# ComputationalRobotics/cuADMM

Measured on NVIDIA B200. Metric: ADMM iterations/s, higher is better.
Workload: dtype f64

## Files before the change

### cuadmm_b200/csrc/dense.cu

```cuda
#include "dense.h"
#include <stdio.h>
#include <stdlib.h>
#include <algorithm>

namespace cuadmm {

static constexpr int GB_M = 64, GB_N = 64, GB_K = 16, GB_PAD = 4;

__device__ __forceinline__ void dmma_m8n8k4(double& c0, double& c1, double a, double b) {
    asm volatile("mma.sync.aligned.m8n8k4.row.col.f64.f64.f64.f64 {%0,%1}, {%2}, {%3}, {%0,%1};"
                 : "+d"(c0), "+d"(c1) : "d"(a), "d"(b));
}

template <bool TA, bool TB>
__global__ void __launch_bounds__(128) dgemm_kernel(int64_t m, int64_t n, int64_t k, double alpha,
                                                    const double* __restrict__ A, int64_t lda,
                                                    const double* __restrict__ B, int64_t ldb,
                                                    double beta, double* C, int64_t ldc, int shape) {
    if (shape == 1 && (int64_t)blockIdx.y * GB_N > (int64_t)blockIdx.x * GB_M + (GB_M - 1)) return;
    __shared__ double As[2][GB_K][GB_M + GB_PAD];
    __shared__ double Bs[2][GB_K][GB_N + GB_PAD];
    const int tid = threadIdx.x, lane = tid & 31, warp = tid >> 5;
    const int wm = (warp & 1) * 32, wn = (warp >> 1) * 32;
    const int64_t m0 = (int64_t)blockIdx.x * GB_M, n0 = (int64_t)blockIdx.y * GB_N;
// ... 108 lines not shown
            for (int t = j; t < i; ++t) s -= S[i][t] * I[t][j];
            I[i][j] = (i >= j) ? s / S[i][i] : 0.0;
        }
    }
    __syncthreads();
    for (int e = tid; e < nb * nb; e += 256) {
        const int i = e % nb, j = e / nb;
        if (i >= j) A[i + j * lda] = S[i][j];
        if (inv) inv[i + (int64_t)j * NB] = I[i][j];
    }
    if (tid == 0 && bad && info) atomicAdd(info, 1);
}

void potrf_lower(cudaStream_t st, int64_t n, double* A, int64_t lda, double* inv_diag, int* d_info, const double* pivot_floor) {
    DevBuf<double> tmp(std::max<int64_t>(n * NB, 1));
    DevBuf<double> inv_local;
    if (!inv_diag) { inv_local.alloc(std::max<int64_t>(n * NB, 1)); inv_diag = inv_local.p; }
    const size_t potf2_bytes = sizeof(double) * 2 * NB * (NB + 1);
    CUADMM_CUDA(cudaFuncSetAttribute((const void*)potf2_inv_kernel, cudaFuncAttributeMaxDynamicSharedMemorySize, (int)potf2_bytes));
    for (int64_t j = 0; j < n; j += NB) {
        const int nb = (int)std::min<int64_t>(NB, n - j);
        double* Ajj = A + j + j * lda;
        double* invj = inv_diag + j * NB;
        potf2_inv_kernel<<<1, 256, potf2_bytes, st>>>(nb, Ajj, lda, invj, d_info, (int)(j / NB), pivot_floor ? pivot_floor + j : nullptr);
        const int64_t below = n - j - nb;
        if (below > 0) {
            double* Aij = A + (j + nb) + j * lda;
            dgemm(st, false, true, below, nb, nb, 1.0, Aij, lda, invj, NB, 0.0, tmp.p, below);
            CUADMM_CUDA(cudaMemcpy2DAsync(Aij, sizeof(double) * lda, tmp.p, sizeof(double) * below,
                                          sizeof(double) * below, nb, cudaMemcpyDeviceToDevice, st));
            double* A22 = A + (j + nb) + (j + nb) * lda;
            dgemm(st, false, true, below, below, nb, -1.0, Aij, lda, Aij, lda, 1.0, A22, lda, 1);
        }
    }
    CUADMM_CUDA(cudaGetLastError());
    CUADMM_CUDA(cudaStreamSynchronize(st));
}

__global__ void copy_inv_block_kernel(int nb, const double* __restrict__ inv, double* X, int64_t ldx) {
    for (int e = threadIdx.x; e < nb * nb; e += blockDim.x) {
        const int i = e % nb, j = e / nb;
        X[i + j * ldx] = inv[i + (int64_t)j * NB];
    }
}

void trtri_lower(cudaStream_t st, int64_t n, const double* L, int64_t ldl, const double* inv_diag, double* X, int64_t ldx) {
    CUADMM_CUDA(cudaMemset2DAsync(X, sizeof(double) * ldx, 0, sizeof(double) * n, n, st));
    DevBuf<double> T(std::max<int64_t>((int64_t)NB * n, 1));
    for (int64_t i = 0; i < n; i += NB) {
        const int nb = (int)std::min<int64_t>(NB, n - i);
        const double* invi = inv_diag + i * NB;
        copy_inv_block_kernel<<<1, 256, 0, st>>>(nb, invi, X + i + i * ldx, ldx);
        if (i > 0) {
            dgemm(st, false, false, nb, i, i, 1.0, L + i, ldl, X, ldx, 0.0, T.p, NB, 2);
            dgemm(st, false, false, nb, i, nb, -1.0, invi, NB, T.p, NB, 0.0, X + i, ldx);
        }
    }
    CUADMM_CUDA(cudaGetLastError());
    CUADMM_CUDA(cudaStreamSynchronize(st));
}

__global__ void scatter_coo_kernel(int64_t nnz, const int32_t* __restrict__ r, const int32_t* __restrict__ c,
                                   const double* __restrict__ v, double* D, int64_t ld, int symmetric) {
    const int64_t e = (int64_t)blockIdx.x * blockDim.x + threadIdx.x;
    if (e >= nnz) return;
    D[r[e] + (int64_t)c[e] * ld] = v[e];
    if (symmetric && r[e] != c[e]) D[c[e] + (int64_t)r[e] * ld] = v[e];
}

__global__ void transpose_kernel(int64_t n, const double* __restrict__ in, double* __restrict__ out) {
    __shared__ double tile[32][33];
    const int64_t bx = (int64_t)blockIdx.x * 32, by = (int64_t)blockIdx.y * 32;
    for (int j = threadIdx.y; j < 32; j += blockDim.y) {
        const int64_t x = bx + threadIdx.x, y = by + j;
        if (x < n && y < n) tile[j][threadIdx.x] = in[x + y * n];
    }
    __syncthreads();
    for (int j = threadIdx.y; j < 32; j += blockDim.y) {
        const int64_t x = by + threadIdx.x, y = bx + j;
        if (x < n && y < n) out[x + y * n] = tile[threadIdx.x][j];
    }
}

__global__ void tile_occupancy_kernel(int64_t r, int nt, const double* __restrict__ A, int* __restrict__ flags) {
    const int I = blockIdx.y, J = blockIdx.x;
    int any = 0;
    for (int e = threadIdx.x; e < 64 * 64; e += blockDim.x) {
        const int64_t i = (int64_t)I * 64 + e / 64, j = (int64_t)J * 64 + e % 64;
        if (i < r && j < r && A[i * r + j] != 0.0) any = 1;
    }
    if (__syncthreads_or(any) && threadIdx.x == 0) flags[I * nt + J] = 1;
}

void build_dense_tail(const SymCsc& C, const CholFactor& F, int64_t n_lead, int64_t r,
                      DevBuf<double>& tail_inv, DevBuf<double>& tail_inv_t, int64_t* n_deficient,
                      std::vector<int>* tile_flags) {
    cudaStream_t st = 0;
    DevBuf<double> S(r * r);
    S.zero(st);
    {
        std::vector<int32_t> rr, cc; std::vector<double> vv;
        for (int64_t j = n_lead; j < n_lead + r; ++j)
            for (int64_t p = C.p[j]; p < C.p[j + 1]; ++p) { rr.push_back((int32_t)(C.i[p] - n_lead)); cc.push_back((int32_t)(j - n_lead)); vv.push_back(C.x[p]); }
        if (!vv.empty()) {
            DevBuf<int32_t> dr, dc; DevBuf<double> dv;
            dr.upload(rr, st); dc.upload(cc, st); dv.upload(vv, st);
            scatter_coo_kernel<<<(unsigned)((vv.size() + 255) / 256), 256, 0, st>>>((int64_t)vv.size(), dr.p, dc.p, dv.p, S.p, r, 1);
            CUADMM_CUDA(cudaStreamSynchronize(st));
        }
    }
    {
        std::vector<int64_t> cols;
        for (int64_t j = 0; j < n_lead; ++j)
            if (F.Lp[j + 1] > F.Lp[j] + 1 && F.Li[F.Lp[j + 1] - 1] >= n_lead) cols.push_back(j);
        const int64_t budget = (int64_t)1 << 27;
        const int64_t cw = std::max<int64_t>(64, std::min<int64_t>((int64_t)cols.size(), budget / std::max<int64_t>(r, 1)));
        DevBuf<double> B(r * std::min<int64_t>(cw, std::max<int64_t>((int64_t)cols.size(), 1)));
        std::vector<int32_t> rr, cc; std::vector<double> vv;
        for (int64_t c0 = 0; c0 < (int64_t)cols.size(); c0 += cw) {
            const int64_t w = std::min<int64_t>(cw, (int64_t)cols.size() - c0);
            rr.clear(); cc.clear(); vv.clear();
            for (int64_t t = 0; t < w; ++t) {
                const int64_t j = cols[c0 + t];
                for (int64_t p = F.Lp[j + 1] - 1; p > F.Lp[j] && F.Li[p] >= n_lead; --p) {
                    rr.push_back((int32_t)(F.Li[p] - n_lead)); cc.push_back((int32_t)t); vv.push_back(F.Lx[p]);
                }
            }
            CUADMM_CUDA(cudaMemsetAsync(B.p, 0, sizeof(double) * (size_t)(r * w), st));
            DevBuf<int32_t> dr, dc; DevBuf<double> dv;
            dr.upload(rr, st); dc.upload(cc, st); dv.upload(vv, st);
            scatter_coo_kernel<<<(unsigned)((vv.size() + 255) / 256), 256, 0, st>>>((int64_t)vv.size(), dr.p, dc.p, dv.p, B.p, r, 0);
            dgemm(st, false, true, r, r, w, -1.0, B.p, r, B.p, r, 1.0, S.p, r, 1);
            CUADMM_CUDA(cudaStreamSynchronize(st));
        }
    }
    DevBuf<double> inv_diag(std::max<int64_t>(r * NB, 1));
    DevBuf<int> info(1);
    info.zero(st);
    std::vector<double> h_floor(r, 0.0);
    for (int64_t j = n_lead; j < n_lead + r; ++j)
        for (int64_t p = C.p[j]; p < C.p[j + 1]; ++p) if (C.i[p] == j) h_floor[j - n_lead] = pivot_tol() * C.x[p];
    DevBuf<double> d_floor; d_floor.upload(h_floor, st);
    potrf_lower(st, r, S.p, r, inv_diag.p, info.p, d_floor.p);
    int h_info = 0;
    info.download(&h_info, 1, st);
    CUADMM_CUDA(cudaStreamSynchronize(st));
    if (n_deficient) *n_deficient = h_info;
    tail_inv_t.alloc(r * r);
    trtri_lower(st, r, S.p, r, inv_diag.p, tail_inv_t.p, r);
    tail_inv.alloc(r * r);
    dim3 grid((unsigned)((r + 31) / 32), (unsigned)((r + 31) / 32)), block(32, 8);
    transpose_kernel<<<grid, block, 0, st>>>(r, tail_inv_t.p, tail_inv.p);
    CUADMM_CUDA(cudaGetLastError());
    CUADMM_CUDA(cudaStreamSynchronize(st));
    {
        const int nt = (int)((r + 63) / 64);
        DevBuf<int> flags((int64_t)nt * nt);
        flags.zero(st);
        tile_occupancy_kernel<<<dim3(nt, nt), 256, 0, st>>>(r, nt, tail_inv.p, flags.p);
        std::vector<int> h((size_t)nt * nt);
        flags.download(h.data(), (int64_t)h.size(), st);
        CUADMM_CUDA(cudaStreamSynchronize(st));
        if (getenv("CUADMM_YSOLVE_VERBOSE")) {
            int64_t lower = 0, used = 0;
            for (int I = 0; I < nt; ++I) for (int J = 0; J <= I; ++J) { ++lower; used += h[(size_t)I * nt + J]; }
            fprintf(stderr, "[ysolve] dense tail %lld: %lld of %lld lower 64x64 tiles of L22^-1 are non-zero (%.1f%%)\n",
                    (long long)r, (long long)used, (long long)lower, 100.0 * (double)used / (double)lower);
        }
        if (tile_flags) tile_flags->swap(h);
    }
}

}
```

### cuadmm_b200/csrc/dense.h

```cpp
#pragma once
#include "common.h"
#include "chol_host.h"

namespace cuadmm {

void dgemm(cudaStream_t st, bool transA, bool transB, int64_t m, int64_t n, int64_t k, double alpha,
           const double* A, int64_t lda, const double* B, int64_t ldb, double beta, double* C, int64_t ldc, int shape = 0);

void potrf_lower(cudaStream_t st, int64_t n, double* A, int64_t lda, double* inv_diag, int* d_info,
                 const double* pivot_floor = nullptr);
void trtri_lower(cudaStream_t st, int64_t n, const double* L, int64_t ldl, const double* inv_diag, double* Linv, int64_t ldi);

void build_dense_tail(const SymCsc& Cperm, const CholFactor& F, int64_t n_lead, int64_t n_tail,
                      DevBuf<double>& tail_inv, DevBuf<double>& tail_inv_t, int64_t* n_deficient = nullptr,
                      std::vector<int>* tile_flags = nullptr);

}
```

### cuadmm_b200/csrc/ysolve.cu

```cuda
#include "ysolve.h"
#include <chrono>
#include <thread>
#include <atomic>
#include "dense.h"
#include <algorithm>
#include <numeric>
#include <stdio.h>
#include <stdlib.h>

namespace cuadmm {

static constexpr int kTriThreads = 256;
static constexpr int kLongRowNnz = 24;
static constexpr int kNarrowSlots = 160;
static constexpr int kNarrowThreads = 1024;

struct SlotWork {
    static constexpr int K = 4;
    int32_t u; int is_long;
    double rv, invd;
    int64_t p, p1; int step;
    int32_t d[K]; double v[K];

    __device__ __forceinline__ void load(int64_t s, int lane, const int32_t* __restrict__ slot_rows,
// ... 265 lines not shown
}

__global__ void __launch_bounds__(kPkThreads, 1) tri_packed_kernel(const int64_t* __restrict__ chunk_off,
        const int64_t* __restrict__ row_off, const unsigned char* __restrict__ stream, const int32_t* __restrict__ prow_u,
        const int32_t* __restrict__ prow_out, const double* __restrict__ w, double* x, double* out_scatter,
        const int* __restrict__ done_flag, long long* __restrict__ timeline) {
    if (done_flag && *done_flag) return;
    if (timeline && threadIdx.x == 0) timeline[4 * blockIdx.x + 0] = pk_globaltimer();
    extern __shared__ __align__(128) unsigned char pk_smem[];
    unsigned char* ring = pk_smem;
    uint64_t* bars = reinterpret_cast<uint64_t*>(pk_smem + kPkRing * kPkChunk);
    double* xs = reinterpret_cast<double*>(pk_smem + kPkRing * kPkChunk + 64);
    const int tid = threadIdx.x, lane = tid & 31, warp = tid >> 5;
    const int64_t c0 = chunk_off[blockIdx.x];
    const int nc = (int)(chunk_off[blockIdx.x + 1] - c0);
    const int64_t r0 = row_off[blockIdx.x];
    const int nr = (int)(row_off[blockIdx.x + 1] - r0);
    const unsigned char* src = stream + c0 * kPkChunk;
    if (tid == 0) {
        for (int i = 0; i < kPkRing; ++i)
            asm volatile("mbarrier.init.shared::cta.b64 [%0], 1;" :: "r"(smem_u32(bars + i)) : "memory");
        asm volatile("fence.mbarrier_init.release.cluster;" ::: "memory");
        asm volatile("fence.proxy.async.shared::cta;" ::: "memory");
        for (int i = 0; i < kPkRing && i < nc; ++i) pk_fetch(ring + i * kPkChunk, src + (int64_t)i * kPkChunk, bars + i);
    }
#pragma unroll 4
    for (int loc = tid; loc < nr; loc += kPkThreads) xs[loc] = w[r0 + loc];
    __syncthreads();
    if (timeline && tid == 0) timeline[4 * blockIdx.x + 1] = pk_globaltimer();
    for (int c = 0; c < nc; ++c) {
        const int b = c % kPkRing;
        pk_wait(bars + b, (uint32_t)((c / kPkRing) & 1));
        pk_chunk<kPkThreads / 32, false>(ring + b * kPkChunk, lane, warp, xs);
        if (tid == 0 && c + kPkRing < nc) pk_fetch(ring + b * kPkChunk, src + (int64_t)(c + kPkRing) * kPkChunk, bars + b);
    }
    if (timeline && tid == 0) timeline[4 * blockIdx.x + 2] = pk_globaltimer();
#pragma unroll 4
    for (int loc = tid; loc < nr; loc += kPkThreads) {
        const int32_t u = prow_u[r0 + loc];
        if (u < 0) continue;
        const double r = xs[loc];
        x[u] = r;
        if (out_scatter) out_scatter[prow_out[r0 + loc]] = r;
    }
    if (timeline && tid == 0) timeline[4 * blockIdx.x + 3] = pk_globaltimer();
}

static constexpr int kPkWarpBlob = 2048;
static constexpr int kPkWarpRows = 32;
static constexpr int kPkWarpThreads = 256;

__global__ void __launch_bounds__(kPkWarpThreads, 5) tri_packed_warp_kernel(int64_t count, const int64_t* __restrict__ blob_off,
        const int64_t* __restrict__ row_off, const uint4* __restrict__ blobs, const int32_t* __restrict__ prow_u,
        const int32_t* __restrict__ prow_out, const double* __restrict__ w, double* x, double* out_scatter,
        const int* __restrict__ done_flag) {
    if (done_flag && *done_flag) return;
    __shared__ __align__(16) unsigned char slices[kPkWarpThreads / 32][kPkWarpBlob];
    __shared__ double xs_all[kPkWarpThreads / 32][kPkWarpRows];
    const int lane = threadIdx.x & 31, warp = threadIdx.x >> 5;
    const int64_t t = (int64_t)blockIdx.x * (kPkWarpThreads / 32) + warp;
    if (t >= count) return;
    const int64_t b0 = blob_off[t];
    const int nb = (int)(blob_off[t + 1] - b0);
    const int64_t r0 = row_off[t];
    const int nr = (int)(row_off[t + 1] - r0);
    uint4* slice = reinterpret_cast<uint4*>(slices[warp]);
    double* xs = xs_all[warp];
    for (int i = lane; i < nb; i += 32) slice[i] = blobs[b0 + i];
    int32_t u = -1, po = -1;
    if (lane < nr) {
        xs[lane] = w[r0 + lane];
        u = prow_u[r0 + lane];
        if (out_scatter) po = prow_out[r0 + lane];
    }
    __syncwarp();
    pk_chunk<1, true>(slices[warp], lane, 0, xs);
    if (lane < nr && u >= 0) {
        const double r = xs[lane];
        x[u] = r;
        if (out_scatter) out_scatter[po] = r;
    }
}

__global__ void __launch_bounds__(256) tail_gemv_row_kernel(int64_t r, const double* __restrict__ T, const double* __restrict__ in,
                                                        double* out, const int32_t* __restrict__ tile_ptr,
                                                        const int32_t* __restrict__ tile_col, double* out_scatter,
                                                        const int32_t* __restrict__ out_perm, int64_t perm_base,
                                                        const int* __restrict__ done_flag, int longest_last) {
    if (done_flag && *done_flag) return;
    const int lane = threadIdx.x & 31;
    const int64_t cta = longest_last ? (int64_t)gridDim.x - 1 - blockIdx.x : blockIdx.x;
    const int64_t row = cta * (blockDim.x >> 5) + (threadIdx.x >> 5);
    if (row >= r) return;
    const double* Ti = T + row * r;
    const int I = (int)(row >> 6);
    double acc0 = 0.0, acc1 = 0.0;
    const bool vec = (r & 1) == 0 && (reinterpret_cast<uintptr_t>(T) & 15) == 0;
    const bool in_al = (reinterpret_cast<uintptr_t>(in) & 15) == 0;
    for (int t = tile_ptr[I]; t < tile_ptr[I + 1]; ++t) {
        const int64_t j0 = tile_col[2 * t];
        const int64_t j1 = min((int64_t)tile_col[2 * t + 1], r);
        if (vec) {
            const int64_t jv = j0 + ((j1 - j0) & ~(int64_t)1);
#pragma unroll 4
            for (int64_t j = j0 + 2 * lane; j < jv; j += 64) {
                const double2 a = __ldcs(reinterpret_cast<const double2*>(Ti + j));
                const double2 b = in_al ? *reinterpret_cast<const double2*>(in + j) : make_double2(in[j], in[j + 1]);
                acc0 = fma(a.x, b.x, acc0);
                acc1 = fma(a.y, b.y, acc1);
            }
            if (lane == 0 && jv < j1) acc0 = fma(Ti[jv], in[jv], acc0);
        } else {
#pragma unroll 4
            for (int64_t j = j0 + lane; j < j1; j += 32) acc0 = fma(Ti[j], in[j], acc0);
        }
    }
    double acc = acc0 + acc1;
#pragma unroll
    for (int o = 16; o > 0; o >>= 1) acc += __shfl_xor_sync(0xffffffffu, acc, o);
    if (lane == 0) {
        out[row] = acc;
        if (out_scatter) out_scatter[out_perm[perm_base + row]] = acc;
    }
}

__global__ void __launch_bounds__(256) tail_gemv_kernel(int64_t r, const double* __restrict__ T, const double* in,
                                                        double* out, const int32_t* __restrict__ tile_ptr,
                                                        const int32_t* __restrict__ tile_col, double* out_scatter,
                                                        const int32_t* __restrict__ out_perm, int64_t perm_base,
                                                        const int* __restrict__ done_flag, int longest_last,
                                                        int64_t row0, int64_t nrows, int npush, PeerView pv,
                                                        PeerPtrs outp, PeerPtrs scatp, int splits, double* split_part,
                                                        unsigned int* split_count) {
    if (done_flag && *done_flag) return;
    __shared__ double part[8][9];
    __shared__ int s_final;
    const int lane = threadIdx.x & 31, w = threadIdx.x >> 5;
    unsigned long long ep = 0;
    if (npush) ep = peer_epoch(pv);
    const int sp = (int)(blockIdx.x % (unsigned)splits);
    const int64_t rb = blockIdx.x / (unsigned)splits, nrb = gridDim.x / (unsigned)splits;
    const int64_t cta = longest_last ? nrb - 1 - rb : rb;
    const int64_t base = row0 + cta * 8;
    const int nr = (int)max((int64_t)0, min((int64_t)8, row0 + nrows - base));
    double acc[8];
#pragma unroll
    for (int q = 0; q < 8; ++q) acc[q] = 0.0;
    if (nr > 0) {
        const int I = (int)(base >> 6);
        const bool vec = (r & 1) == 0 && (reinterpret_cast<uintptr_t>(T) & 15) == 0 && (reinterpret_cast<uintptr_t>(in) & 15) == 0;
        const double* Tb = T + base * r;
        int g = 0;
        for (int t = tile_ptr[I]; t < tile_ptr[I + 1]; ++t) {
            const int64_t j0 = tile_col[2 * t];
            const int64_t j1 = min((int64_t)tile_col[2 * t + 1], r);
            const int nch = (int)((j1 - j0 + 63) >> 6);
            const int g0 = g;
            int c = (w - (g & 7)) & 7;
            g += nch;
            for (; c < nch; c += 8) {
                if (splits > 1 && (((g0 + c) >> 3) % splits) != sp) continue;
                const int64_t j = j0 + ((int64_t)c << 6) + 2 * lane;
                if (vec) {
                    if (j + 1 < j1) {
                        const double2 b = *reinterpret_cast<const double2*>(in + j);
#pragma unroll
                        for (int q = 0; q < 8; ++q) {
                            if (q < nr) {
                                const double2 a = __ldcs(reinterpret_cast<const double2*>(Tb + q * r + j));
                                acc[q] = fma(a.x, b.x, fma(a.y, b.y, acc[q]));
                            }
                        }
                    } else if (j < j1) {
                        const double b = in[j];
#pragma unroll
                        for (int q = 0; q < 8; ++q) if (q < nr) acc[q] = fma(Tb[q * r + j], b, acc[q]);
                    }
                } else {
#pragma unroll
                    for (int h = 0; h < 2; ++h) {
                        const int64_t jj = j0 + ((int64_t)c << 6) + lane + 32 * h;
                        if (jj < j1) {
                            const double b = in[jj];
#pragma unroll
                            for (int q = 0; q < 8; ++q) if (q < nr) acc[q] = fma(Tb[q * r + jj], b, acc[q]);
                        }
                    }
                }
            }
        }
    }
#pragma unroll
    for (int q = 0; q < 8; ++q) {
#pragma unroll
        for (int o = 16; o > 0; o >>= 1) acc[q] += __shfl_xor_sync(0xffffffffu, acc[q], o);
    }
    if (lane == 0) {
#pragma unroll
        for (int q = 0; q < 8; ++q) part[w][q] = acc[q];
    }
    __syncthreads();
    const int t = threadIdx.x;
    bool final_cta = true;
    if (splits > 1) {
        if (t < 8) {
// ... 484 lines not shown
            for (int64_t t = 0; t < H.n_sub; ++t) {
                const int64_t sz = (int64_t)members[t].size();
                if (sz <= edges[b] && (b == 0 || sz > edges[b - 1])) { ++cnt; r += sz; dsum += depth[t]; dmax = std::max(dmax, depth[t]); }
            }
            if (cnt) fprintf(stderr, "[ysolve]   rows<=%lld: %lld subtrees, %lld rows, sum depth %lld, max depth %d\n",
                             (long long)edges[b], (long long)cnt, (long long)r, (long long)dsum, dmax);
        }
    }
    int maxlev = -1;
    for (int32_t u : H.order) if (H.sub[u] < 0) maxlev = std::max(maxlev, (int)level[u]);
    S.levels = maxlev + 1;
    std::vector<std::vector<int32_t>> top_by_level(std::max(S.levels, 0));
    for (int32_t u : H.order) if (H.sub[u] < 0) top_by_level[level[u]].push_back(u);
    S.h_level_ptr.assign(S.levels + 1, (int64_t)slot_info.size());
    std::vector<int64_t> level_slots(std::max(S.levels, 1), 0);
    for (int l = 0; l < S.levels; ++l) {
        S.h_level_ptr[l] = (int64_t)slot_info.size();
        level_slots[l] = emit_level_slots(H, top_by_level[l], l, slot_rows, slot_info);
        S.h_level_ptr[l + 1] = (int64_t)slot_info.size();
    }
    S.n_slots = (int64_t)slot_info.size();
    int narrow_slots = kNarrowSlots;
    if (const char* e = getenv("CUADMM_SWEEP_NARROW_SLOTS")) narrow_slots = atoi(e);
    S.phases.clear();
    for (int l = 0; l < S.levels;) {
        if (level_slots[l] <= narrow_slots) {
            int e = l;
            while (e < S.levels && level_slots[e] <= narrow_slots) ++e;
            S.phases.push_back({true, l, e});
            l = e;
        } else {
            S.phases.push_back({false, l, l + 1});
            ++l;
        }
    }
    S.ptr.upload(H.ptr);
    std::vector<int32_t> dep(H.dep); if (dep.empty()) dep.push_back(0);
    std::vector<double> val(H.val); if (val.empty()) val.push_back(0.0);
    S.dep.upload(dep); S.val.upload(val);
    S.inv_diag.upload(H.inv_diag);
    if (slot_rows.empty()) { slot_rows.assign(8, -1); slot_info.push_back(0); }
    S.slot_rows.upload(slot_rows); S.slot_info.upload(slot_info);
    S.level_ptr.upload(S.h_level_ptr);
    if (sub_lvl_ptr.empty()) sub_lvl_ptr.push_back(0);
    S.sub_off.upload(sub_off); S.sub_lvl_ptr.upload(sub_lvl_ptr);
}

static int64_t choose_subtrees(const CholFactor& F, int64_t n_lead, std::vector<int32_t>& sub) {
    const int64_t n = F.n;
    sub.assign(n, -1);
    int64_t cap = 12000;
    if (const char* e = getenv("CUADMM_SWEEP_SUBTREE_CAP")) cap = atoll(e);
    if (cap <= 0) return 0;
    cap = std::min<int64_t>(cap, (int64_t)(232448 - kPkRing * kPkChunk - 64) / 8 - kPkChainMax);
    int64_t min_size = 2;
    if (const char* e = getenv("CUADMM_SWEEP_SUBTREE_MIN")) min_size = atoll(e);
    std::vector<int64_t> size(n, 1);
    for (int64_t v = 0; v < n_lead; ++v) {
        const int32_t p = F.parent[v];
        if (p >= 0 && p < n_lead) size[p] += size[v];
    }
    int64_t n_sub = 0;
    for (int64_t v = n_lead - 1; v >= 0; --v) {
        const int32_t p = F.parent[v];
        const bool parent_top = (p < 0 || p >= n_lead || sub[p] < 0);
        if (!parent_top) { sub[v] = sub[p]; continue; }
        const bool parent_fits = (p >= 0 && p < n_lead && size[p] <= cap);
        if (size[v] <= cap && !parent_fits && size[v] >= min_size) sub[v] = (int32_t)n_sub++;
    }
    return n_sub;
}

static int64_t choose_tail(const CholFactor& F, std::vector<int32_t>& level_out) {
    const int64_t n = F.n;
    std::vector<int32_t> lev(n, 0);
    for (int64_t j = 0; j < n; ++j)
        for (int64_t p = F.Lp[j] + 1; p < F.Lp[j + 1]; ++p) lev[F.Li[p]] = std::max(lev[F.Li[p]], lev[j] + 1);
    level_out = lev;
    int depth = 0;
    for (int64_t i = 0; i < n; ++i) depth = std::max(depth, lev[i] + 1);
    int64_t max_tail = 10240;
    int min_depth = 64;
    if (const char* e = getenv("CUADMM_YSOLVE_MAX_TAIL")) max_tail = atoll(e);
    if (const char* e = getenv("CUADMM_YSOLVE_MIN_DEPTH")) min_depth = atoi(e);
    if (depth <= min_depth || max_tail <= 0) return depth + 1;
    std::vector<int64_t> cnt(depth + 1, 0);
    for (int64_t i = 0; i < n; ++i) cnt[lev[i]]++;
    int64_t above = 0;
    int cut = depth;
    for (int l = depth - 1; l >= min_depth / 2; --l) {
        if (above + cnt[l] > max_tail) break;
        above += cnt[l];
        cut = l;
    }
    if (above < 32) return depth + 1;
    return cut;
}

cuadmm_ysolve_s* ysolve_create(int64_t m, int64_t vec_len, int64_t nnz, const int32_t* rowptr, const int32_t* colind,
                               const double* val, double eps, int device) {
    CUADMM_REQUIRE(m >= 0 && vec_len >= 0 && nnz >= 0, "negative dimension");
    CUADMM_REQUIRE(rowptr && (nnz == 0 || (colind && val)), "null argument");
    CUADMM_REQUIRE(rowptr[0] == 0 && rowptr[m] == nnz, "rowptr does not span nnz");
    int cnt = 0;
    if (cudaGetDeviceCount(&cnt) != cudaSuccess || cnt == 0) {
        cudaGetLastError();
        throw Error(CUADMM_ENODEVICE, "no CUDA device available; the y-solve has no CPU fallback");
    }
    CUADMM_REQUIRE(device >= 0 && device < cnt, "device index out of range");
    std::unique_ptr<cuadmm_ysolve_s> Y(new cuadmm_ysolve_s());
    Y->device = device; Y->m = m;
    DeviceGuard g(device);

    const bool vtime = getenv("CUADMM_YSOLVE_VERBOSE") != nullptr;
    auto tp0 = std::chrono::steady_clock::now();
    auto lap = [&](const char* what) {
        if (!vtime) return;
        const auto t = std::chrono::steady_clock::now();
        fprintf(stderr, "[ysolve] init %-28s %8.1f ms\n", what, std::chrono::duration<double, std::milli>(t - tp0).count());
        tp0 = t;
    };
    SymCsc M = form_aat(m, vec_len, rowptr, colind, val, eps);
    lap("A A^T");
    Y->nnz_aat = M.p[m];
    std::vector<int32_t> perm0 = min_degree_order(M);
    lap("minimum-degree ordering");
    CholFactor F;
    chol_symbolic(M, perm0, F, nullptr);
    lap("symbolic (1)");
    std::vector<int32_t> lev;
    const int64_t cut = choose_tail(F, lev);
    std::vector<int32_t> perm1; perm1.reserve(m);
    for (int64_t k = 0; k < m; ++k) if (lev[k] < cut) perm1.push_back(F.perm[k]);
    const int64_t n_lead = (int64_t)perm1.size();
    for (int64_t k = 0; k < m; ++k) if (lev[k] >= cut) perm1.push_back(F.perm[k]);
    const int64_t n_tail = m - n_lead;
    SymCsc C;
    if (n_tail > 0) {
        F = CholFactor();
        chol_symbolic(M, perm1, F, &C);
    } else {
        chol_symbolic(M, perm0, F, &C);
    }
    lap("symbolic (2, tail last)");
    chol_numeric(C, F, n_lead);
    lap("numeric (sparse lead part)");
    Y->n_lead = n_lead; Y->n_tail = n_tail;
    Y->nnz_L = F.nnz();
    Y->n_deficient = F.n_deficient;
    Y->h_perm = F.perm;
    Y->perm.upload(F.perm);

    std::vector<int32_t> sub;
    const int64_t n_sub = choose_subtrees(F, n_lead, sub);
    {
        HostSweep H;
        H.n = m;
        H.ptr.assign(m + 1, 0);
        for (int64_t j = 0; j < n_lead; ++j)
            for (int64_t p = F.Lp[j] + 1; p < F.Lp[j + 1]; ++p) H.ptr[F.Li[p] + 1]++;
        for (int64_t i = 0; i < m; ++i) H.ptr[i + 1] += H.ptr[i];
        H.dep.resize(H.ptr[m]); H.val.resize(H.ptr[m]);
        std::vector<int64_t> nx(H.ptr.begin(), H.ptr.end() - 1);
        for (int64_t j = 0; j < n_lead; ++j)
            for (int64_t p = F.Lp[j] + 1; p < F.Lp[j + 1]; ++p) {
                const int64_t q = nx[F.Li[p]]++;
                H.dep[q] = (int32_t)j; H.val[q] = F.Lx[p];
            }
        H.inv_diag.assign(m, 1.0);
        for (int64_t i = 0; i < n_lead; ++i) H.inv_diag[i] = 1.0 / F.Lx[F.Lp[i]];
        H.order.resize(m);
        std::iota(H.order.begin(), H.order.end(), 0);
        H.sub = sub; H.n_sub = n_sub; H.subtrees_first = true;
        H.gather = &Y->h_perm;
        upload_sweep(H, Y->fwd);
    }
    {
        HostSweep H;
        H.n = m;
        H.ptr.assign(m + 1, 0);
        for (int64_t j = 0; j < n_lead; ++j) H.ptr[j + 1] = F.Lp[j + 1] - F.Lp[j] - 1;
        for (int64_t i = 0; i < m; ++i) H.ptr[i + 1] += H.ptr[i];
        H.dep.resize(H.ptr[m]); H.val.resize(H.ptr[m]);
        for (int64_t j = 0; j < n_lead; ++j) {
            int64_t q = H.ptr[j];
            for (int64_t p = F.Lp[j] + 1; p < F.Lp[j + 1]; ++p, ++q) { H.dep[q] = F.Li[p]; H.val[q] = F.Lx[p]; }
        }
        H.inv_diag.assign(m, 1.0);
        for (int64_t i = 0; i < n_lead; ++i) H.inv_diag[i] = 1.0 / F.Lx[F.Lp[i]];
        H.order.resize(n_lead);
        for (int64_t j = 0; j < n_lead; ++j) H.order[j] = (int32_t)(n_lead - 1 - j);
        H.sub = sub;
        for (int64_t i = n_lead; i < m; ++i) H.sub[i] = -2;
        H.n_sub = n_sub; H.subtrees_first = false;
        H.out_perm = &Y->h_perm;
        upload_sweep(H, Y->bwd);
    }
    lap("pack + upload sweeps");
    Y->z.alloc(std::max<int64_t>(m, 1));
    Y->x.alloc(std::max<int64_t>(m, 1));

    if (n_tail > 0) {
        int64_t tail_def = 0;
        std::vector<int> flags;
        build_dense_tail(C, F, n_lead, n_tail, Y->tail_inv, Y->tail_inv_t, &tail_def, &flags);
        const int nt = (int)((n_tail + 63) / 64);
        std::vector<int32_t> tp(1, 0), tc, tpt(1, 0), tct;
        auto add_runs = [&](std::vector<int32_t>& ptr, std::vector<int32_t>& col, int J0, int J1, auto used) {
            for (int J = J0; J < J1;) {
                if (!used(J)) { ++J; continue; }
                int E = J;
                while (E < J1 && used(E)) ++E;
                col.push_back(J * 64); col.push_back(E * 64);
                J = E;
            }
            ptr.push_back((int32_t)(col.size() / 2));
        };
        Y->h_tail_cost[0].assign(nt, 0.0); Y->h_tail_cost[1].assign(nt, 0.0);
        for (int I = 0; I < nt; ++I) {
            add_runs(tp, tc, 0, I + 1, [&](int J) { return flags[(size_t)I * nt + J] != 0; });
            add_runs(tpt, tct, I, nt, [&](int J) { return flags[(size_t)J * nt + I] != 0; });
            for (int32_t t = tp[I]; t < tp[I + 1]; ++t) Y->h_tail_cost[0][I] += tc[2 * t + 1] - tc[2 * t];
            for (int32_t t = tpt[I]; t < tpt[I + 1]; ++t) Y->h_tail_cost[1][I] += tct[2 * t + 1] - tct[2 * t];
        }
        if (tc.empty()) tc.assign(2, 0);
        if (tct.empty()) tct.assign(2, 0);
        Y->tail_tptr.upload(tp); Y->tail_tcol.upload(tc); Y->tail_tptr_t.upload(tpt); Y->tail_tcol_t.upload(tct);
        Y->n_deficient += tail_def;
        Y->tail_tmp.alloc(n_tail);
        lap("dense tail (GPU)");
    }
    Y->launches_per_solve = (int)(Y->fwd.phases.size() + Y->bwd.phases.size()) + (n_tail > 0 ? 2 : 0) +
                            (Y->fwd.n_sub_cta > 0 ? 2 : 0) + (Y->fwd.n_sub_warp > 0 ? 2 : 0) + (Y->fwd.n_sub_pack > 0 ? 2 : 0) +
                            (Y->fwd.pk_rows > 0 ? 2 : 0);
    CUADMM_CUDA(cudaStreamCreateWithFlags(&Y->streams.side, cudaStreamNonBlocking));
    CUADMM_CUDA(cudaEventCreateWithFlags(&Y->streams.fork, cudaEventDisableTiming));
    CUADMM_CUDA(cudaEventCreateWithFlags(&Y->streams.join, cudaEventDisableTiming));
    Y->alg_bytes = 2 * (12 * Y->nnz_L + 8 * m) + 24 * m;
    CUADMM_CUDA(cudaDeviceSynchronize());
    return Y.release();
}

}

using namespace cuadmm;

cuadmm_ysolve_s::~cuadmm_ysolve_s() {
    if (streams.fork) cudaEventDestroy(streams.fork);
    if (streams.join) cudaEventDestroy(streams.join);
    if (streams.side) cudaStreamDestroy(streams.side);
}

void cuadmm_ysolve_s::enable_peer(const PeerComm* pc, size_t off_tmp, size_t off_x) {
    peer = pc;
    peer_tmp = pc->ptrs(off_tmp);
    peer_x = pc->ptrs(off_x);
    tail_tmp_p = pc->local<double>(off_tmp);
    x_p = pc->local<double>(off_x);
    if (n_tail > 0 && pc->world > 1) launches_per_solve += 1;
    split_tail_rows(pc->world, pc->rank);
}

void cuadmm_ysolve_s::split_tail_rows(int world, int rank) {
    for (int k = 0; k < 2; ++k) {
        const std::vector<double>& c = h_tail_cost[k];
        double total = 0.0;
        for (int64_t i = 0; i < n_tail; ++i) total += c[i >> 6] + 32.0;
        std::vector<int64_t> cut(world + 1, n_tail);
        cut[0] = 0;
        double acc = 0.0;
        int q = 1;
        for (int64_t i = 0; i < n_tail && q < world; ++i) {
            acc += c[i >> 6] + 32.0;
            while (q < world && acc >= total * q / world) cut[q++] = std::min<int64_t>(n_tail, (i + 1 + 7) / 8 * 8);
        }
        tail_row0[k] = cut[rank]; tail_row1[k] = cut[rank + 1];
    }
    const int64_t nrb = std::max<int64_t>(1, (std::max(tail_row1[0] - tail_row0[0], tail_row1[1] - tail_row0[1]) + 7) / 8);
    split_part.alloc(nrb * 8 * 8);
    split_count.alloc(nrb);
    split_count.zero();
    CUADMM_CUDA(cudaDeviceSynchronize());
}

void cuadmm_ysolve_s::solve(const double* d_rhs_, double* d_y_, cudaStream_t st) {
    if (m == 0) return;
    double* xv = x_p ? x_p : x.p;
    double* tmpv = tail_tmp_p ? tail_tmp_p : tail_tmp.p;
    launch_sweep(fwd, d_rhs_, perm.p, z.p, nullptr, nullptr, done_flag, st, streams);
    auto mark = [&](int tag) {
        if (!prof_ev) return;
        cudaEvent_t ev;
        CUADMM_CUDA(cudaEventCreate(&ev));
        CUADMM_CUDA(cudaEventRecord(ev, st));
        prof_ev->push_back(ev); prof_tag->push_back(tag);
    };
    auto gemv_split = [&](const double* Tm, const double* in, double* out, const int32_t* tp, const int32_t* tc, int longest_last,
                          int64_t r0, int64_t nrows_, int npush, const PeerView& pv, const PeerPtrs& outp) {
        const int64_t nrb = std::max<int64_t>(1, (nrows_ + 7) / 8);
        int splits = (int)std::min<int64_t>(8, std::max<int64_t>(1, (2 * 148 + nrb - 1) / nrb));
        CUADMM_REQUIRE(split_part.n >= nrb * 8 * 8 && split_count.n >= nrb, "internal: split-column GEMV scratch too small");
        tail_gemv_kernel<<<(unsigned)(nrb * splits), 256, 0, st>>>(n_tail, Tm, in, out, tp, tc, nullptr, nullptr, 0, done_flag,
            longest_last, r0, nrows_, npush, pv, outp, PeerPtrs(), splits, split_part.p, split_count.p);
    };
    if (n_tail > 0) {
        mark(20);
        if (!peer || peer->world == 1) {
            const int blocks = (int)((n_tail + 7) / 8);
            tail_gemv_row_kernel<<<blocks, 256, 0, st>>>(n_tail, tail_inv.p, z.p + n_lead, tmpv, tail_tptr.p, tail_tcol.p,
                                                         nullptr, nullptr, 0, done_flag, 1);
            tail_gemv_row_kernel<<<blocks, 256, 0, st>>>(n_tail, tail_inv_t.p, tmpv, xv + n_lead, tail_tptr_t.p, tail_tcol_t.p,
                                                         d_y_, perm.p, n_lead, done_flag, 0);
        } else {
            PeerPtrs pxt = peer_x;
            for (int q = 0; q < peer->world; ++q) pxt.p[q] += n_lead;
            const PeerView pv = peer->view();
            const int64_t n0 = tail_row1[0] - tail_row0[0], n1 = tail_row1[1] - tail_row0[1];
            gemv_split(tail_inv.p, z.p + n_lead, tmpv, tail_tptr.p, tail_tcol.p, 1, tail_row0[0], n0, peer->world, pv, peer_tmp);
            gemv_split(tail_inv_t.p, tmpv, xv + n_lead, tail_tptr_t.p, tail_tcol_t.p, 0, tail_row0[1], n1, peer->world, pv, pxt);
            tail_scatter_kernel<<<(int)((n_tail + 255) / 256), 256, 0, st>>>(n_tail, xv + n_lead, perm.p, n_lead, d_y_, done_flag);
        }
        CUADMM_CUDA(cudaGetLastError());
        mark(21);
    }
    launch_sweep(bwd, z.p, nullptr, xv, d_y_, perm.p, done_flag, st, streams);
}

extern "C" {

int cuadmm_ysolve_create(int64_t m, int64_t vec_len, int64_t nnz, const int32_t* h_A_rowptr, const int32_t* h_A_colind,
                         const double* h_A_val, double eps, int device, cuadmm_ysolve_t** out) {
    return guarded([&] {
        CUADMM_REQUIRE(out != nullptr, "out is null");
        *out = nullptr;
        *out = ysolve_create(m, vec_len, nnz, h_A_rowptr, h_A_colind, h_A_val, eps, device);
    });
}

void cuadmm_ysolve_destroy(cuadmm_ysolve_t* ys) { delete ys; }

int cuadmm_ysolve(cuadmm_ysolve_t* ys, const double* d_rhs, double* d_y, void* stream) {
    return guarded([&] {
        CUADMM_REQUIRE(ys && d_rhs && d_y, "null argument");
        DeviceGuard g(ys->device);
        ys->solve(d_rhs, d_y, (cudaStream_t)stream);
    });
}

int cuadmm_debug_ysolve_timeline(cuadmm_ysolve_t* ys, int which, long long* timeline, long long* meta, int64_t cap, int64_t* n) {
    return guarded([&] {
        CUADMM_REQUIRE(ys && n, "null argument");
        DeviceGuard g(ys->device);
        const cuadmm::TriSweep& S = which ? ys->bwd : ys->fwd;
        *n = S.pk_timeline.n / 4;
        if (!timeline || cap < *n || *n == 0) return;
        CUADMM_CUDA(cudaDeviceSynchronize());
        CUADMM_CUDA(cudaMemcpy(timeline, S.pk_timeline.p, sizeof(long long) * 4 * (size_t)*n, cudaMemcpyDeviceToHost));
        if (meta) std::copy(S.pk_timeline_meta.begin(), S.pk_timeline_meta.end(), meta);
    });
}

int cuadmm_ysolve_host(cuadmm_ysolve_t* ys, const double* h_rhs, double* h_y) {
    return guarded([&] {
        CUADMM_REQUIRE(ys && h_rhs && h_y, "null argument");
        DeviceGuard g(ys->device);
        if (ys->d_rhs.n != ys->m) { ys->d_rhs.alloc(std::max<int64_t>(ys->m, 1)); ys->d_y.alloc(std::max<int64_t>(ys->m, 1)); }
        ys->d_rhs.upload(h_rhs, ys->m);
        ys->solve(ys->d_rhs.p, ys->d_y.p, 0);
        ys->d_y.download(h_y, ys->m);
        CUADMM_CUDA(cudaStreamSynchronize(0));
    });
}

int cuadmm_ysolve_stats(const cuadmm_ysolve_t* ys, int64_t out[8]) {
    return guarded([&] {
        CUADMM_REQUIRE(ys && out, "null argument");
        out[0] = ys->nnz_aat; out[1] = ys->nnz_L; out[2] = std::max(ys->fwd.levels, ys->bwd.levels);
        out[3] = ys->n_tail; out[4] = ys->launches_per_solve; out[5] = ys->alg_bytes;
        out[6] = ys->n_deficient; out[7] = ys->fwd.n_sub * 100000 + ys->fwd.sub_depth;
    });
}

int cuadmm_ysolve_perm(const cuadmm_ysolve_t* ys, int32_t* perm) {
    return guarded([&] {
        CUADMM_REQUIRE(ys && perm, "null argument");
        std::copy(ys->h_perm.begin(), ys->h_perm.end(), perm);
    });
}

}
```

### cuadmm_b200/csrc/ysolve.h

```cpp
#pragma once
#include "common.h"
#include "chol_host.h"
#include "peer.h"

namespace cuadmm {

struct TriSweep {
    int64_t n_unknowns = 0;
    int64_t nnz = 0;
    DevBuf<int64_t> ptr;
    DevBuf<int32_t> dep;
    DevBuf<double> val;
    DevBuf<double> inv_diag;
    DevBuf<int32_t> slot_rows;
    DevBuf<int32_t> slot_info;
    DevBuf<int64_t> level_ptr;
    std::vector<int64_t> h_level_ptr;
    struct Phase { bool narrow; int level0, level1; };
    std::vector<Phase> phases;
    int64_t n_slots = 0;
    int levels = 0;
    DevBuf<int64_t> sub_off, sub_lvl_ptr;
    int64_t n_sub = 0;
    int64_t n_sub_cta = 0;
    int64_t n_sub_pack = 0, n_sub_warp = 0, pk_rows = 0;
    DevBuf<unsigned char> pk_stream, pk_blobs;
    DevBuf<int64_t> pk_chunk_off, pk_blob_off, pk_row_off, pk_ext_ptr;
    DevBuf<int32_t> pk_prow_u, pk_prow_src, pk_prow_out, pk_ext_dep, pk_heavy;
    int64_t pk_n_heavy = 0;
    DevBuf<double> pk_ext_val, pk_w;
    DevBuf<long long> pk_timeline;
    std::vector<long long> pk_timeline_meta;
    size_t pk_smem = 0;
    bool pk_has_ext = false;
    int sub_depth = 0;
    bool subtrees_first = true;
};

struct SweepStreams {
    cudaStream_t side = nullptr;
    cudaEvent_t fork = nullptr, join = nullptr;
};

}

struct cuadmm_ysolve_s {
    int device = -1;
    int64_t m = 0;
    int64_t n_lead = 0, n_tail = 0;
    int64_t nnz_aat = 0, nnz_L = 0, n_deficient = 0;
    cuadmm::TriSweep fwd, bwd;
    cuadmm::DevBuf<int32_t> perm;
    cuadmm::DevBuf<double> z;
    cuadmm::DevBuf<double> x;
    cuadmm::DevBuf<double> tail_inv, tail_inv_t, tail_tmp;
    cuadmm::DevBuf<int32_t> tail_tptr, tail_tcol, tail_tptr_t, tail_tcol_t;
    cuadmm::DevBuf<double> d_rhs, d_y;
    std::vector<int32_t> h_perm;
    const cuadmm::PeerComm* peer = nullptr;
    double* tail_tmp_p = nullptr;
    double* x_p = nullptr;
    cuadmm::PeerPtrs peer_tmp, peer_x;
    int64_t tail_row0[2] = {0, 0}, tail_row1[2] = {0, 0};
    std::vector<double> h_tail_cost[2];
    void enable_peer(const cuadmm::PeerComm* pc, size_t off_tmp, size_t off_x);
    void split_tail_rows(int world, int rank);
    cuadmm::DevBuf<double> split_part;
    cuadmm::DevBuf<unsigned int> split_count;
    const int* done_flag = nullptr;
    std::vector<cudaEvent_t>* prof_ev = nullptr;
    std::vector<int>* prof_tag = nullptr;
    cuadmm::SweepStreams streams;
    ~cuadmm_ysolve_s();
    int launches_per_solve = 0;
    int64_t alg_bytes = 0;
    void solve(const double* d_rhs, double* d_y, cudaStream_t stream);
};

namespace cuadmm {
cuadmm_ysolve_s* ysolve_create(int64_t m, int64_t vec_len, int64_t nnz, const int32_t* rowptr, const int32_t* colind,
                               const double* val, double eps, int device);
}
```

Baseline: 833.6.

## Fuse dense tail forward/backward GEMVs into one row-batched kernel reading W once

Replaces the two row-wise GEMV passes over the dense tail inverse and its transpose with a single persistent kernel. Each block owns a cost-balanced band of rows, computes t = W z for a small batch of rows, then immediately applies W^T t to a shared-memory partial x while the rows are still hot. A second small kernel sums the per-group partials and scatters the result into y. The aim is to read the dense inverse roughly once per solve instead of twice, and to drop the transposed copy in the single-GPU case. The cost is a per-group partial buffer, a reduction pass, large shared-memory use per block, and a cap on the tail size.

Result: slower. 707.8, median of 6 (-15.1%).

```diff
diff --git a/cuadmm_b200/csrc/dense.cu b/cuadmm_b200/csrc/dense.cu
--- a/cuadmm_b200/csrc/dense.cu
+++ b/cuadmm_b200/csrc/dense.cu
@@ -214,6 +214,12 @@
     }
 }
 
+void transpose_dense(int64_t n, const double* in, double* out, cudaStream_t st) {
+    dim3 grid((unsigned)((n + 31) / 32), (unsigned)((n + 31) / 32)), block(32, 8);
+    transpose_kernel<<<grid, block, 0, st>>>(n, in, out);
+    CUADMM_CUDA(cudaGetLastError());
+}
+
 __global__ void tile_occupancy_kernel(int64_t r, int nt, const double* __restrict__ A, int* __restrict__ flags) {
     const int I = blockIdx.y, J = blockIdx.x;
     int any = 0;
@@ -225,8 +231,7 @@
 }
 
 void build_dense_tail(const SymCsc& C, const CholFactor& F, int64_t n_lead, int64_t r,
-                      DevBuf<double>& tail_inv, DevBuf<double>& tail_inv_t, int64_t* n_deficient,
-                      std::vector<int>* tile_flags) {
+                      DevBuf<double>& tail_inv, int64_t* n_deficient, std::vector<int>* tile_flags) {
     cudaStream_t st = 0;
     DevBuf<double> S(r * r);
     S.zero(st);
@@ -278,13 +283,13 @@
     info.download(&h_info, 1, st);
     CUADMM_CUDA(cudaStreamSynchronize(st));
     if (n_deficient) *n_deficient = h_info;
-    tail_inv_t.alloc(r * r);
-    trtri_lower(st, r, S.p, r, inv_diag.p, tail_inv_t.p, r);
-    tail_inv.alloc(r * r);
-    dim3 grid((unsigned)((r + 31) / 32), (unsigned)((r + 31) / 32)), block(32, 8);
-    transpose_kernel<<<grid, block, 0, st>>>(r, tail_inv_t.p, tail_inv.p);
-    CUADMM_CUDA(cudaGetLastError());
-    CUADMM_CUDA(cudaStreamSynchronize(st));
+    {
+        DevBuf<double> inv_cm(r * r);
+        trtri_lower(st, r, S.p, r, inv_diag.p, inv_cm.p, r);
+        tail_inv.alloc(r * r);
+        transpose_dense(r, inv_cm.p, tail_inv.p, st);
+        CUADMM_CUDA(cudaStreamSynchronize(st));
+    }
     {
         const int nt = (int)((r + 63) / 64);
         DevBuf<int> flags((int64_t)nt * nt);
diff --git a/cuadmm_b200/csrc/dense.h b/cuadmm_b200/csrc/dense.h
--- a/cuadmm_b200/csrc/dense.h
+++ b/cuadmm_b200/csrc/dense.h
@@ -11,8 +11,10 @@
                  const double* pivot_floor = nullptr);
 void trtri_lower(cudaStream_t st, int64_t n, const double* L, int64_t ldl, const double* inv_diag, double* Linv, int64_t ldi);
 
+void transpose_dense(int64_t n, const double* in, double* out, cudaStream_t st);
+
 void build_dense_tail(const SymCsc& Cperm, const CholFactor& F, int64_t n_lead, int64_t n_tail,
-                      DevBuf<double>& tail_inv, DevBuf<double>& tail_inv_t, int64_t* n_deficient = nullptr,
+                      DevBuf<double>& tail_inv, int64_t* n_deficient = nullptr,
                       std::vector<int>* tile_flags = nullptr);
 
 }
diff --git a/cuadmm_b200/csrc/ysolve.cu b/cuadmm_b200/csrc/ysolve.cu
--- a/cuadmm_b200/csrc/ysolve.cu
+++ b/cuadmm_b200/csrc/ysolve.cu
@@ -371,45 +371,191 @@
     }
 }
 
-__global__ void __launch_bounds__(256) tail_gemv_row_kernel(int64_t r, const double* __restrict__ T, const double* __restrict__ in,
-                                                        double* out, const int32_t* __restrict__ tile_ptr,
-                                                        const int32_t* __restrict__ tile_col, double* out_scatter,
-                                                        const int32_t* __restrict__ out_perm, int64_t perm_base,
-                                                        const int* __restrict__ done_flag, int longest_last) {
+static constexpr int kTailThreads = 256;
+static constexpr int kTailWarps = kTailThreads / 32;
+static constexpr int kTailChunks = 3;
+static constexpr int kTailGroups = 148;
+static constexpr int64_t kTailBatchBytes = 256 << 10;
+static constexpr double kTailBatchCost = 8192.0;
+static constexpr int64_t kTailMaxRows = 13824;
+
+static inline size_t tail_solve_smem(int64_t len) {
+    return sizeof(double) * (size_t)(2 * ((len + 1) & ~(int64_t)1) + kTailWarps * 8 + 64 + 2 * kTailThreads);
+}
+
+template <bool kStream>
+__device__ __forceinline__ double2 tail_pair(const double* p, bool vec, bool two) {
+    if (vec) return kStream ? __ldcs(reinterpret_cast<const double2*>(p)) : __ldg(reinterpret_cast<const double2*>(p));
+    return make_double2(p[0], two ? p[1] : 0.0);
+}
+
+__global__ void __launch_bounds__(kTailThreads, 1) tail_solve_kernel(int64_t r, const double* __restrict__ W,
+        const double* __restrict__ z, const int32_t* __restrict__ tile_ptr, const int32_t* __restrict__ tile_col,
+        const int2* __restrict__ batch, const int32_t* __restrict__ batch_ptr, const int32_t* __restrict__ glen,
+        double* __restrict__ part, const int* __restrict__ done_flag) {
     if (done_flag && *done_flag) return;
-    const int lane = threadIdx.x & 31;
-    const int64_t cta = longest_last ? (int64_t)gridDim.x - 1 - blockIdx.x : blockIdx.x;
-    const int64_t row = cta * (blockDim.x >> 5) + (threadIdx.x >> 5);
-    if (row >= r) return;
-    const double* Ti = T + row * r;
-    const int I = (int)(row >> 6);
-    double acc0 = 0.0, acc1 = 0.0;
-    const bool vec = (r & 1) == 0 && (reinterpret_cast<uintptr_t>(T) & 15) == 0;
-    const bool in_al = (reinterpret_cast<uintptr_t>(in) & 15) == 0;
-    for (int t = tile_ptr[I]; t < tile_ptr[I + 1]; ++t) {
-        const int64_t j0 = tile_col[2 * t];
-        const int64_t j1 = min((int64_t)tile_col[2 * t + 1], r);
-        if (vec) {
-            const int64_t jv = j0 + ((j1 - j0) & ~(int64_t)1);
+    extern __shared__ __align__(16) double tail_sm[];
+    const int g = blockIdx.x;
+    const int64_t L = glen[g];
+    double* zs = tail_sm;
+    double* xs = zs + ((L + 1) & ~(int64_t)1);
+    double* wp = xs + ((L + 1) & ~(int64_t)1);
+    double* ts = wp + kTailWarps * 8;
+    double* red = ts + 64;
+    const int tid = threadIdx.x, lane = tid & 31, warp = tid >> 5;
+    for (int64_t j = tid; j < L; j += kTailThreads) { zs[j] = z[j]; xs[j] = 0.0; }
+    const bool vec = (r & 1) == 0 && (reinterpret_cast<uintptr_t>(W) & 15) == 0;
+    __syncthreads();
+    for (int b = batch_ptr[g]; b < batch_ptr[g + 1]; ++b) {
+        const int64_t row0 = batch[b].x;
+        const int nr = batch[b].y;
+        const int I = (int)(row0 >> 6);
+        const int t0 = tile_ptr[I], t1 = tile_ptr[I + 1];
+        const int noct = nr <= 8 ? 1 : nr <= 16 ? 2 : nr <= 32 ? 4 : 8;
+        const int wpo = kTailWarps / noct;
+        const int o = warp / wpo, sub = warp % wpo;
+        const int nro = max(0, min(8, nr - 8 * o));
+        const double* Wo = W + (row0 + 8 * o) * r;
+        double acc[8];
+#pragma unroll
+        for (int q = 0; q < 8; ++q) acc[q] = 0.0;
+        if (nro > 0) {
+            int gc = 0;
+            for (int t = t0; t < t1; ++t) {
+                const int64_t j0 = tile_col[2 * t];
+                const int64_t j1 = min((int64_t)tile_col[2 * t + 1], r);
+                const int nch = (int)((j1 - j0 + 63) >> 6);
+                int c = ((sub - gc) % wpo + wpo) % wpo;
+                gc += nch;
+                for (; c < nch; c += kTailChunks * wpo) {
+                    double2 a[kTailChunks][8], zz[kTailChunks];
+#pragma unroll
+                    for (int u = 0; u < kTailChunks; ++u) {
+                        const int64_t j = j0 + ((int64_t)(c + u * wpo) << 6) + 2 * lane;
+                        const bool v = c + u * wpo < nch && j < j1, two = j + 1 < j1;
+#pragma unroll
+                        for (int q = 0; q < 8; ++q)
+                            if (q < nro) a[u][q] = v ? tail_pair<false>(Wo + q * r + j, vec, two) : make_double2(0.0, 0.0);
+                        zz[u] = !v ? make_double2(0.0, 0.0) : vec ? *reinterpret_cast<const double2*>(zs + j)
+                                                             : make_double2(zs[j], two ? zs[j + 1] : 0.0);
+                    }
+#pragma unroll
+                    for (int u = 0; u < kTailChunks; ++u) {
+#pragma unroll
+                        for (int q = 0; q < 8; ++q)
+                            if (q < nro) acc[q] = fma(a[u][q].x, zz[u].x, fma(a[u][q].y, zz[u].y, acc[q]));
+                    }
+                }
+            }
+        }
+#pragma unroll
+        for (int q = 0; q < 8; ++q) {
+#pragma unroll
+            for (int s = 16; s > 0; s >>= 1) acc[q] += __shfl_xor_sync(0xffffffffu, acc[q], s);
+        }
+        if (lane == 0) {
+#pragma unroll
+            for (int q = 0; q < 8; ++q) wp[warp * 8 + q] = acc[q];
+        }
+        __syncthreads();
+        if (tid < nr) {
+            const int oo = tid >> 3, q = tid & 7;
+            double v = 0.0;
+            for (int s = 0; s < wpo; ++s) v += wp[(oo * wpo + s) * 8 + q];
+            ts[tid] = v;
+        }
+        __syncthreads();
+        int npair = 0;
+        for (int t = t0; t < t1; ++t) npair += (int)((min((int64_t)tile_col[2 * t + 1], r) - tile_col[2 * t] + 1) >> 1);
+        int S = 1;
+        while (S < 8 && 2 * S <= nr && 2 * S * npair <= kTailThreads) S *= 2;
+        const int tp = kTailThreads / S, sl = tid / tp, pi = tid % tp;
+        const int qa = sl * nr / S, qb = (sl + 1) * nr / S;
+        const double* Wb = W + row0 * r;
+        auto locate = [&](int k, int64_t& j, int64_t& j1) {
+            for (int t = t0; t < t1; ++t) {
+                const int64_t c0 = tile_col[2 * t], c1 = min((int64_t)tile_col[2 * t + 1], r);
+                const int np = (int)((c1 - c0 + 1) >> 1);
+                if (k < np) { j = c0 + 2 * k; j1 = c1; return; }
+                k -= np;
+            }
+        };
+        for (int k = pi; k < npair; k += 2 * tp) {
+            const bool hb = k + tp < npair;
+            int64_t ja = 0, j1a = 0, jb = 0, j1b = 0;
+            locate(k, ja, j1a);
+            if (hb) locate(k + tp, jb, j1b);
+            const bool twa = ja + 1 < j1a, twb = jb + 1 < j1b;
+            double xa0 = 0.0, xa1 = 0.0, xb0 = 0.0, xb1 = 0.0;
+            if (sl == 0) {
+                xa0 = xs[ja]; xa1 = twa ? xs[ja + 1] : 0.0;
+                if (hb) { xb0 = xs[jb]; xb1 = twb ? xs[jb + 1] : 0.0; }
+            }
+            for (int q0 = qa; q0 < qb; q0 += 8) {
+                double2 va[8], vb[8];
+#pragma unroll
+                for (int q = 0; q < 8; ++q) {
+                    if (q0 + q < qb) {
+                        va[q] = tail_pair<true>(Wb + (int64_t)(q0 + q) * r + ja, vec, twa);
+                        if (hb) vb[q] = tail_pair<true>(Wb + (int64_t)(q0 + q) * r + jb, vec, twb);
+                    }
+                }
+#pragma unroll
+                for (int q = 0; q < 8; ++q) {
+                    if (q0 + q < qb) {
+                        const double tq = ts[q0 + q];
+                        xa0 = fma(va[q].x, tq, xa0);
+                        xa1 = fma(va[q].y, tq, xa1);
+                        if (hb) { xb0 = fma(vb[q].x, tq, xb0); xb1 = fma(vb[q].y, tq, xb1); }
+                    }
+                }
+            }
+            if (S == 1) {
+                xs[ja] = xa0;
+                if (twa) xs[ja + 1] = xa1;
+                if (hb) { xs[jb] = xb0; if (twb) xs[jb + 1] = xb1; }
+            } else {
+                red[2 * tid] = xa0; red[2 * tid + 1] = xa1;
+            }
+        }
+        if (S > 1) {
+            __syncthreads();
+            if (tid < npair) {
+                double x0 = red[2 * tid], x1 = red[2 * tid + 1];
+                for (int q = 1; q < S; ++q) { x0 += red[2 * (q * tp + tid)]; x1 += red[2 * (q * tp + tid) + 1]; }
+                int64_t j = 0, j1 = 0;
+                locate(tid, j, j1);
+                xs[j] = x0;
+                if (j + 1 < j1) xs[j + 1] = x1;
+            }
+        }
+    }
+    __syncthreads();
+    double* pg = part + (int64_t)g * r;
+    for (int64_t j = tid; j < L; j += kTailThreads) pg[j] = xs[j];
+}
+
+__global__ void __launch_bounds__(256) tail_reduce_kernel(int64_t r, int G, const double* __restrict__ part,
+        const int32_t* __restrict__ glen, double* __restrict__ out, double* __restrict__ y,
+        const int32_t* __restrict__ perm, int64_t perm_base, const int* __restrict__ done_flag) {
+    if (done_flag && *done_flag) return;
+    __shared__ double sh[8][33];
+    const int lane = threadIdx.x & 31, w = threadIdx.x >> 5;
+    const int64_t j = (int64_t)blockIdx.x * 32 + lane;
+    double v = 0.0;
+    if (j < r) {
 #pragma unroll 4
-            for (int64_t j = j0 + 2 * lane; j < jv; j += 64) {
-                const double2 a = __ldcs(reinterpret_cast<const double2*>(Ti + j));
-                const double2 b = in_al ? *reinterpret_cast<const double2*>(in + j) : make_double2(in[j], in[j + 1]);
-                acc0 = fma(a.x, b.x, acc0);
-                acc1 = fma(a.y, b.y, acc1);
-            }
-            if (lane == 0 && jv < j1) acc0 = fma(Ti[jv], in[jv], acc0);
-        } else {
-#pragma unroll 4
-            for (int64_t j = j0 + lane; j < j1; j += 32) acc0 = fma(Ti[j], in[j], acc0);
-        }
-    }
-    double acc = acc0 + acc1;
-#pragma unroll
-    for (int o = 16; o > 0; o >>= 1) acc += __shfl_xor_sync(0xffffffffu, acc, o);
-    if (lane == 0) {
-        out[row] = acc;
-        if (out_scatter) out_scatter[out_perm[perm_base + row]] = acc;
+        for (int g = w; g < G; g += 8)
+            if (__ldg(glen + g) > j) v += __ldcg(part + (int64_t)g * r + j);
+    }
+    sh[w][lane] = v;
+    __syncthreads();
+    if (w == 0 && j < r) {
+        double s = 0.0;
+#pragma unroll
+        for (int k = 0; k < 8; ++k) s += sh[k][lane];
+        out[j] = s;
+        y[perm[perm_base + j]] = s;
     }
 }
 
@@ -1060,6 +1206,7 @@
     int64_t max_tail = 10240;
     int min_depth = 64;
     if (const char* e = getenv("CUADMM_YSOLVE_MAX_TAIL")) max_tail = atoll(e);
+    max_tail = std::min(max_tail, kTailMaxRows);
     if (const char* e = getenv("CUADMM_YSOLVE_MIN_DEPTH")) min_depth = atoi(e);
     if (depth <= min_depth || max_tail <= 0) return depth + 1;
     std::vector<int64_t> cnt(depth + 1, 0);
@@ -1181,7 +1328,7 @@
     if (n_tail > 0) {
         int64_t tail_def = 0;
         std::vector<int> flags;
-        build_dense_tail(C, F, n_lead, n_tail, Y->tail_inv, Y->tail_inv_t, &tail_def, &flags);
+        build_dense_tail(C, F, n_lead, n_tail, Y->tail_inv, &tail_def, &flags);
         const int nt = (int)((n_tail + 63) / 64);
         std::vector<int32_t> tp(1, 0), tc, tpt(1, 0), tct;
         auto add_runs = [&](std::vector<int32_t>& ptr, std::vector<int32_t>& col, int J0, int J1, auto used) {
@@ -1205,7 +1352,7 @@
         if (tct.empty()) tct.assign(2, 0);
         Y->tail_tptr.upload(tp); Y->tail_tcol.upload(tc); Y->tail_tptr_t.upload(tpt); Y->tail_tcol_t.upload(tct);
         Y->n_deficient += tail_def;
-        Y->tail_tmp.alloc(n_tail);
+        Y->plan_tail_groups();
         lap("dense tail (GPU)");
     }
     Y->launches_per_solve = (int)(Y->fwd.phases.size() + Y->bwd.phases.size()) + (n_tail > 0 ? 2 : 0) +
@@ -1235,8 +1382,54 @@
     peer_x = pc->ptrs(off_x);
     tail_tmp_p = pc->local<double>(off_tmp);
     x_p = pc->local<double>(off_x);
-    if (n_tail > 0 && pc->world > 1) launches_per_solve += 1;
+    if (n_tail > 0 && pc->world > 1) {
+        launches_per_solve += 1;
+        tail_inv_t.alloc(n_tail * n_tail);
+        transpose_dense(n_tail, tail_inv.p, tail_inv_t.p, 0);
+    }
     split_tail_rows(pc->world, pc->rank);
+}
+
+void cuadmm_ysolve_s::plan_tail_groups() {
+    const std::vector<double>& c = h_tail_cost[0];
+    const int G = (int)std::min<int64_t>(kTailGroups, (n_tail + 7) / 8);
+    auto batch_rows = [&](int64_t I) {
+        int64_t rows = 8;
+        while (rows < 64 && 2 * rows * (int64_t)c[I] * 8 <= kTailBatchBytes) rows *= 2;
+        return rows;
+    };
+    auto row_cost = [&](int64_t i) { return c[i >> 6] + 32.0 + kTailBatchCost / (double)batch_rows(i >> 6); };
+    double total = 0.0;
+    for (int64_t i = 0; i < n_tail; ++i) total += row_cost(i);
+    std::vector<int64_t> cut(G + 1, n_tail);
+    cut[0] = 0;
+    double acc = 0.0;
+    int q = 1;
+    for (int64_t i = 0; i < n_tail && q < G; ++i) {
+        acc += row_cost(i);
+        while (q < G && acc >= total * q / G) cut[q++] = std::min<int64_t>(n_tail, (i + 1 + 7) / 8 * 8);
+    }
+    std::vector<int2> bt;
+    std::vector<int32_t> bp(1, 0), gl(G, 0);
+    int64_t len_max = 0;
+    for (int k = 0; k < G; ++k) {
+        for (int64_t i = cut[k]; i < cut[k + 1];) {
+            const int64_t I = i >> 6;
+            const int64_t rows = std::min({batch_rows(I), (I + 1) * 64 - i, cut[k + 1] - i});
+            bt.push_back(make_int2((int)i, (int)rows));
+            i += rows;
+        }
+        bp.push_back((int32_t)bt.size());
+        if (cut[k + 1] > cut[k]) gl[k] = (int32_t)std::min<int64_t>(n_tail, (cut[k + 1] + 63) / 64 * 64);
+        len_max = std::max<int64_t>(len_max, gl[k]);
+    }
+    if (bt.empty()) bt.push_back(make_int2(0, 0));
+    tail_groups = G;
+    tail_smem = tail_solve_smem(len_max);
+    tail_batch.upload(bt); tail_bptr.upload(bp); tail_glen.upload(gl);
+    tail_part.alloc((int64_t)G * n_tail);
+    CUADMM_CUDA(cudaFuncSetAttribute(tail_solve_kernel, cudaFuncAttributeMaxDynamicSharedMemorySize,
+                                     (int)tail_solve_smem(kTailMaxRows)));
 }
 
 void cuadmm_ysolve_s::split_tail_rows(int world, int rank) {
@@ -1264,7 +1457,6 @@
 void cuadmm_ysolve_s::solve(const double* d_rhs_, double* d_y_, cudaStream_t st) {
     if (m == 0) return;
     double* xv = x_p ? x_p : x.p;
-    double* tmpv = tail_tmp_p ? tail_tmp_p : tail_tmp.p;
     launch_sweep(fwd, d_rhs_, perm.p, z.p, nullptr, nullptr, done_flag, st, streams);
     auto mark = [&](int tag) {
         if (!prof_ev) return;
@@ -1284,12 +1476,12 @@
     if (n_tail > 0) {
         mark(20);
         if (!peer || peer->world == 1) {
-            const int blocks = (int)((n_tail + 7) / 8);
-            tail_gemv_row_kernel<<<blocks, 256, 0, st>>>(n_tail, tail_inv.p, z.p + n_lead, tmpv, tail_tptr.p, tail_tcol.p,
-                                                         nullptr, nullptr, 0, done_flag, 1);
-            tail_gemv_row_kernel<<<blocks, 256, 0, st>>>(n_tail, tail_inv_t.p, tmpv, xv + n_lead, tail_tptr_t.p, tail_tcol_t.p,
-                                                         d_y_, perm.p, n_lead, done_flag, 0);
+            tail_solve_kernel<<<tail_groups, kTailThreads, tail_smem, st>>>(n_tail, tail_inv.p, z.p + n_lead, tail_tptr.p,
+                tail_tcol.p, tail_batch.p, tail_bptr.p, tail_glen.p, tail_part.p, done_flag);
+            tail_reduce_kernel<<<(unsigned)((n_tail + 31) / 32), 256, 0, st>>>(n_tail, tail_groups, tail_part.p, tail_glen.p,
+                xv + n_lead, d_y_, perm.p, n_lead, done_flag);
         } else {
+            double* tmpv = tail_tmp_p;
             PeerPtrs pxt = peer_x;
             for (int q = 0; q < peer->world; ++q) pxt.p[q] += n_lead;
             const PeerView pv = peer->view();
diff --git a/cuadmm_b200/csrc/ysolve.h b/cuadmm_b200/csrc/ysolve.h
--- a/cuadmm_b200/csrc/ysolve.h
+++ b/cuadmm_b200/csrc/ysolve.h
@@ -53,8 +53,14 @@
     cuadmm::DevBuf<int32_t> perm;
     cuadmm::DevBuf<double> z;
     cuadmm::DevBuf<double> x;
-    cuadmm::DevBuf<double> tail_inv, tail_inv_t, tail_tmp;
+    cuadmm::DevBuf<double> tail_inv, tail_inv_t;
     cuadmm::DevBuf<int32_t> tail_tptr, tail_tcol, tail_tptr_t, tail_tcol_t;
+    int tail_groups = 0;
+    size_t tail_smem = 0;
+    cuadmm::DevBuf<int2> tail_batch;
+    cuadmm::DevBuf<int32_t> tail_bptr, tail_glen;
+    cuadmm::DevBuf<double> tail_part;
+    void plan_tail_groups();
     cuadmm::DevBuf<double> d_rhs, d_y;
     std::vector<int32_t> h_perm;
     const cuadmm::PeerComm* peer = nullptr;
```
